# mederrata/spmf

Hardware: AMD Instinct MI355X
Metric: elbo_steps_per_sec (higher is better)
Workload: dtype f32

## Files before the change

### spmf_amd/csrc/common.h

```cpp
#pragma once
#include <hip/hip_runtime.h>
#include <stdint.h>

#define SPMF_WAVE 64

namespace spmf {

constexpr double kHalfLog2OverPi = -0.22579135264472743236;
constexpr double kLgammaHalf = 0.57236494292470008707;
constexpr double kLog2 = 0.69314718055994530942;

constexpr int kDaccHead = 6;
constexpr int kDaccDynSlot = 5;
__host__ __device__ constexpr bool lik_exp(int l) { return l == 1 || l == 4; }
__host__ __device__ constexpr bool lik_bern(int l) { return l == 2 || l == 4; }

constexpr float kYSat = 70.0f;
__device__ __forceinline__ float expm1_dec(float y, float& ey) {
  float p = 1.f / 40320.f;
  p = fmaf(p, y, 1.f / 5040.f);
  p = fmaf(p, y, 1.f / 720.f);
  p = fmaf(p, y, 1.f / 120.f);
  p = fmaf(p, y, 1.f / 24.f);
  p = fmaf(p, y, 1.f / 6.f);
  p = fmaf(p, y, 0.5f);
  p = fmaf(p, y, 1.f);
  const float e = expf(y);
  const bool small = fabsf(y) < 0.25f;
  const float em1 = small ? y * p : e - 1.f;
  ey = small ? 1.f + em1 : e;
  return em1;
}

__device__ __forceinline__ float cell_softplus(float r) { return fmaxf(r, 0.f) + log1pf(expf(-fabsf(r))); }
__device__ __forceinline__ bool cell_is_bern(int lik, const uint8_t* __restrict__ ctype, int d) {
  return lik_bern(lik) || (lik == 3 && ctype[d]);
}
__device__ __forceinline__ float cell_rate(int lik, float y, const float& phi, float& ey) {
  ey = 1.f;
  return (lik_exp(lik) ? expm1_dec(fminf(y, kYSat), ey) : y) + phi;
}
__device__ __forceinline__ float cell_ll0(bool bern, float r) { return bern ? -cell_softplus(r) : -r; }
template <bool LGAMMA>
__device__ __forceinline__ float cell_ll(bool bern, float x, float r) {
  if (bern) return x * r - cell_softplus(r);
  const float xl = x == 0.f ? 0.f : x * logf(r);
  return LGAMMA ? xl - lgammaf(x + 1.f) - r : xl - r;
}
__device__ __forceinline__ float cell_mean(bool bern, float r) {
  if (!bern) return r;
  const float e = expf(-fabsf(r));
  const float p = 1.f / (1.f + e);
  return r >= 0.f ? p : e * p;
}
__device__ __forceinline__ void lse_update(float ll, float& m, float& se) {
  const float d = ll - m;
  const float e = expf(-fabsf(d));
  se = d > 0.f ? fmaf(se, e, 1.f) : se + e;
  m = fmaxf(m, ll);
}

constexpr int kPrepSeg = 8;
#ifndef FINISH_FTD
#define FINISH_FTD 32
#endif
constexpr int kFinishCols = FINISH_FTD;
constexpr int kDaccRep = 16;
constexpr int kDetMaxBlocks = 4096;
constexpr int kDetMeta = 8;
__host__ __device__ inline int det_part_len(int KP) { return 2 * KP + 4; }

__host__ __device__ inline int acc_tail_len(int KP) { return 2 * (kDaccHead + KP); }
struct AccLayout {
  int D, KP, Dh;
  __host__ __device__ int64_t half_len(int h) const {
    return (int64_t)(h ? D - Dh : Dh) * (2 * KP + 1);
  }
  __host__ __device__ int64_t gA_off(int h) const { return h ? half_len(0) - (int64_t)Dh * KP : 0; }
  __host__ __device__ int64_t gV_off(int h) const {
    return h ? half_len(0) + (int64_t)(D - Dh) * KP - (int64_t)Dh * KP : (int64_t)Dh * KP;
  }
  __host__ __device__ int64_t gphi_off(int h) const {
    return h ? half_len(0) + (int64_t)2 * (D - Dh) * KP - Dh : (int64_t)2 * Dh * KP;
  }
  __host__ __device__ int64_t tail_off() const { return (int64_t)2 * D * KP + D; }
};
__host__ __device__ inline int64_t acc_len(int D, int KP) {
  return (int64_t)2 * D * KP + D + acc_tail_len(KP);
}

__device__ __forceinline__ void fold_dacc(int i, const double* __restrict__ dacc, float* __restrict__ tail, int KP) {
  double v = 0.0;
  if (i != kDaccDynSlot) {
#pragma unroll
    for (int r = 0; r < kDaccRep; ++r) v += dacc[(size_t)r * (kDaccHead + KP) + i];
  }
  const float hi = (float)v;
  tail[2 * i] = hi;
  tail[2 * i + 1] = (float)(v - (double)hi);
}

__device__ __forceinline__ double prep_sum(const double* __restrict__ dprep, int KP, int i) {
  double t = 0.0;
#pragma unroll
  for (int g = 0; g < kPrepSeg; ++g) t += dprep[(size_t)g * (KP + 1) + i];
  return t;
}

__device__ __forceinline__ float4 shfl4(float4 v, int src) {
  return make_float4(__shfl(v.x, src), __shfl(v.y, src), __shfl(v.z, src), __shfl(v.w, src));
}
__device__ __forceinline__ float4 shfl_xor4(float4 v, int m) {
  return make_float4(__shfl_xor(v.x, m), __shfl_xor(v.y, m), __shfl_xor(v.z, m),
                     __shfl_xor(v.w, m));
}
__device__ __forceinline__ float4 add4(float4 a, float4 b) {
  return make_float4(a.x + b.x, a.y + b.y, a.z + b.z, a.w + b.w);
}
__device__ __forceinline__ float4 fma4(float s, float4 a, float4 acc) {
  return make_float4(fmaf(s, a.x, acc.x), fmaf(s, a.y, acc.y), fmaf(s, a.z, acc.z),
                     fmaf(s, a.w, acc.w));
}
__device__ __forceinline__ float dot4(float4 a, float4 b) {
  return fmaf(a.x, b.x, fmaf(a.y, b.y, fmaf(a.z, b.z, a.w * b.w)));
}

template <int LPN>
__device__ __forceinline__ float4 gather4(const float* __restrict__ base, int row, int sub) {
  const uint32_t off = ((uint32_t)row * (uint32_t)LPN + (uint32_t)sub) * 16u;
  return *reinterpret_cast<const float4*>(reinterpret_cast<const char*>(base) + off);
}

constexpr int kPadRow = -1;
constexpr uint32_t kPadWord = 0xffff0000u;
struct GTable {
  __amdgpu_buffer_rsrc_t r;
};
__device__ __forceinline__ GTable gtable(const float* base, int64_t rows, int KP) {
  GTable t;
  t.r = __builtin_amdgcn_make_buffer_rsrc(const_cast<float*>(base), 0, (int)(uint32_t)((uint64_t)rows * KP * 4u),
                                          0x00020000);
  return t;
}
template <int LPN>
__device__ __forceinline__ float4 gather4(const GTable& t, int row, int sub) {
  const uint32_t off = ((uint32_t)row * (uint32_t)LPN + (uint32_t)sub) * 16u;
  typedef unsigned int u4 __attribute__((ext_vector_type(4)));
  const u4 v = __builtin_amdgcn_raw_buffer_load_b128(t.r, (int)off, 0, 0);
  return make_float4(__uint_as_float(v.x), __uint_as_float(v.y), __uint_as_float(v.z), __uint_as_float(v.w));
}

template <int CTRL>
__device__ __forceinline__ float dpp_add(float v) {
  const int t = __builtin_amdgcn_update_dpp(0, __float_as_int(v), CTRL, 0xF, 0xF, true);
  return v + __int_as_float(t);
}
template <int N>
__device__ __forceinline__ float group_sum(float v) {
  if constexpr (N >= 2) v = dpp_add<0xB1>(v);
  if constexpr (N >= 4) v = dpp_add<0x4E>(v);
  if constexpr (N >= 8) v = dpp_add<0x141>(v);
  if constexpr (N >= 16) v = dpp_add<0x140>(v);
  return v;
}
template <int LPN>
__device__ __forceinline__ float across_groups_sum(float v) {
  if constexpr (LPN <= 1) v = dpp_add<0x121>(v);
  if constexpr (LPN <= 2) v = dpp_add<0x122>(v);
  if constexpr (LPN <= 4) v = dpp_add<0x124>(v);
  if constexpr (LPN <= 8) v = dpp_add<0x128>(v);
  v += __shfl_xor(v, 16);
  v += __shfl_xor(v, 32);
  return v;
}
template <int LPN>
__device__ __forceinline__ float4 across_groups_sum4(float4 v) {
  return make_float4(across_groups_sum<LPN>(v.x), across_groups_sum<LPN>(v.y),
                     across_groups_sum<LPN>(v.z), across_groups_sum<LPN>(v.w));
}

__device__ __forceinline__ double wave_sum(double v) {
#pragma unroll
  for (int m = 32; m >= 1; m >>= 1) v += __shfl_xor(v, m);
  return v;
}
__device__ __forceinline__ float wave_sum(float v) {
#pragma unroll
  for (int m = 32; m >= 1; m >>= 1) v += __shfl_xor(v, m);
  return v;
}

__device__ __forceinline__ double block_sum(double v, double* red) {
  v = wave_sum(v);
  const int wid = threadIdx.x >> 6, lane = threadIdx.x & 63;
  const int nw = (blockDim.x + 63) >> 6;
  __syncthreads();
  if (lane == 0) red[wid] = v;
  __syncthreads();
  double t = 0.0;
  if (threadIdx.x == 0)
    for (int i = 0; i < nw; ++i) t += red[i];
  return t;
}

}
```

### spmf_amd/csrc/row_pass.hip

```cpp
#include <algorithm>

#include "common.h"
#include "kernels.h"

namespace spmf {

#ifndef ROW_MAX_BLOCKS
#define ROW_MAX_BLOCKS 4096
#endif
#ifndef ROW_DYN_NUM
#define ROW_DYN_NUM 1
#define ROW_DYN_DEN 8
#endif
static_assert(ROW_MAX_BLOCKS <= spmf::kDetMaxBlocks,
              "the deterministic mode's per-workgroup slots (common.h kDetMaxBlocks) are sized for at most that many row-pass workgroups");
#ifndef ROW_GRP
#define ROW_GRP 4
#endif
#ifndef ROW_V_AHEAD
#define ROW_V_AHEAD 2
#endif
#ifndef ROW_WAVES_PER_SIMD
#define ROW_WAVES_PER_SIMD 1
#endif

namespace {

__device__ __forceinline__ float* lds_dyn() {
  extern __shared__ __attribute__((aligned(16))) float spmf_row_lds[];
  return spmf_row_lds;
}

template <int FMT, bool NT>
__device__ __forceinline__ void load_entry(const int32_t* __restrict__ col, const float* __restrict__ val,
                                           const uint32_t* __restrict__ ent, int i, bool ok, int& ra,
                                           float& rb) {
  if (FMT == 1) {
    ra = ok ? (int)(NT ? __builtin_nontemporal_load(&ent[i]) : ent[i]) : (int)kPadWord;
    rb = 0.f;
  } else {
    ra = ok ? (NT ? __builtin_nontemporal_load(&col[i]) : col[i]) : kPadRow;
    rb = ok ? (NT ? __builtin_nontemporal_load(&val[i]) : val[i]) : 0.f;
  }
}
template <int FMT>
__device__ __forceinline__ void unpack_entry(int ra, float rb, int& c, float& x) {
  if (FMT == 1) {
    c = (int)((uint32_t)ra >> 16);
    x = (float)((uint32_t)ra & 0xffffu);
  } else {
    c = ra;
    x = rb;
  }
}

template <bool BASE>
__device__ __forceinline__ int bperm_i(int base_bytes, int imm_lanes, int v) {
  if constexpr (BASE) return __builtin_amdgcn_ds_bpermute(base_bytes + imm_lanes * 4, v);
  else return __shfl(v, (base_bytes >> 2) + imm_lanes);
}
template <bool BASE>
__device__ __forceinline__ float bperm_f(int base_bytes, int imm_lanes, float v) {
  return __int_as_float(bperm_i<BASE>(base_bytes, imm_lanes, __float_as_int(v)));
}

template <int KP, int LIK, bool LDSPHI = false>
struct RowCtx {
  static constexpr int LPN = KP / 4;
  static constexpr int NPI = 64 / LPN;
  static constexpr int GRP = LPN < ROW_GRP ? LPN : ROW_GRP;
  static constexpr bool BPI = LPN <= 8 && LIK != 1;
  GTable Ap, Vp;
  const float* phi;
  const uint8_t* ctype;
  int lane, sub, grp;
  int bp_grp, bp_row;

  template <int CNT>
  __device__ __forceinline__ void s1_group(int c, float x, int g0, float4& zacc) const {
    float4 a[CNT];
    float xv[CNT];
#pragma unroll
    for (int j = 0; j < CNT; ++j) {
      const int d = bperm_i<BPI>(bp_grp, (g0 + j) * NPI, c);
      xv[j] = bperm_f<BPI>(bp_grp, (g0 + j) * NPI, x);
      a[j] = gather4<LPN>(Ap, d, sub);
    }
#pragma unroll
    for (int j = 0; j < CNT; ++j) zacc = fma4(xv[j], a[j], zacc);
  }
  __device__ __forceinline__ void sweep1(int c, float x, int nchunk, float4& zacc) const {
#pragma unroll
    for (int g0 = 0; g0 < LPN; g0 += GRP) {
      if (g0 * NPI < nchunk) s1_group<GRP>(c, x, g0, zacc);
    }
  }

  template <int CNT>
  __device__ __forceinline__ void s2_gather(int c, int g0, const float4& z, float4 (&vv)[LPN],
                                            float& rmine) const {
#pragma unroll
    for (int j = 0; j < CNT; ++j) {
      const int d = bperm_i<BPI>(bp_grp, (g0 + j) * NPI, c);
      vv[g0 + j] = gather4<LPN>(Vp, d, sub);
    }
#pragma unroll
    for (int j = 0; j < CNT; ++j) {
      const float dot = group_sum<LPN>(dot4(z, vv[g0 + j]));
      if (sub == g0 + j) rmine = dot;
    }
#pragma unroll
    for (int j = CNT; j < GRP; ++j) vv[g0 + j] = make_float4(0.f, 0.f, 0.f, 0.f);
  }
  template <int CNT>
  __device__ __forceinline__ void s2_back(float cc, int g0, const float4 (&vv)[LPN],
                                          float4& gz) const {
#pragma unroll
    for (int j = 0; j < CNT; ++j) {
      const float cb = bperm_f<BPI>(bp_row, g0 + j, cc);
      gz = fma4(cb, vv[g0 + j], gz);
    }
  }

  __device__ __forceinline__ void s2_load(int c, int nchunk, float4 (&vv)[LPN]) const {
#pragma unroll
    for (int g0 = 0; g0 < LPN; g0 += GRP) {
      if (g0 * NPI < nchunk) {
#pragma unroll
        for (int j = 0; j < GRP; ++j) {
          const int d = bperm_i<BPI>(bp_grp, (g0 + j) * NPI, c);
          vv[g0 + j] = gather4<LPN>(Vp, d, sub);
        }
      } else {
#pragma unroll
        for (int j = 0; j < GRP; ++j) vv[g0 + j] = make_float4(0.f, 0.f, 0.f, 0.f);
      }
    }
  }
  __device__ __forceinline__ void sweep2_loaded(int c, float x, int nchunk, const float4& z, float4& gz, float& ll,
                                                double& nnf, const float4 (&vv)[LPN]) const {
    float rmine = 0.f;
#pragma unroll
    for (int g0 = 0; g0 < LPN; g0 += GRP) {
      if (g0 * NPI < nchunk) {
#pragma unroll
        for (int j = 0; j < GRP; ++j) {
          const float dot = group_sum<LPN>(dot4(z, vv[g0 + j]));
          if (sub == g0 + j) rmine = dot;
        }
      }
    }
    s2_cells(c, x, nchunk, rmine, vv, gz, ll, nnf);
  }

  __device__ __forceinline__ void sweep2(int c, float x, int nchunk, const float4& z,
                                         float4& gz, float& ll, double& nnf) const {
    float4 vv[LPN];
    float rmine = 0.f;
#pragma unroll
    for (int g0 = 0; g0 < LPN; g0 += GRP) {
      if (g0 * NPI < nchunk) s2_gather<GRP>(c, g0, z, vv, rmine);
      else s2_gather<0>(c, g0, z, vv, rmine);
    }
    s2_cells(c, x, nchunk, rmine, vv, gz, ll, nnf);
  }
  __device__ __forceinline__ void s2_cells(int c, float x, int nchunk, float rmine, const float4 (&vv)[LPN],
                                           float4& gz, float& ll, double& nnf) const {
    const int slot = sub * NPI + grp;
    const float xs = __shfl(x, slot);
    const int cs = __shfl(c, slot);
    float cc = 0.f;
    if (slot < nchunk && xs > 0.f) {
      if (LIK == 2 || LIK == 4 || (LIK == 3 && ctype[cs])) {
        float ey = 1.f;
        const float fy = LIK == 4 ? expm1_dec(fminf(rmine, kYSat), ey) : rmine;
        const float lg = fy + (LDSPHI ? lds_dyn()[cs] : phi[cs]);
        if (lg > -INFINITY && lg < INFINITY) {
          ll = fmaf(xs, lg, ll);
          cc = LIK == 4 ? xs * ey : xs;
        } else {
          nnf += 1.0;
        }
      } else {
        float ey = 1.f;
        const float fy = LIK == 1 ? expm1_dec(fminf(rmine, kYSat), ey) : rmine;
        const float r = fy + (LDSPHI ? lds_dyn()[cs] : phi[cs]);
        if (r > 0.f && r < INFINITY) {
          ll = fmaf(xs, logf(r), ll);
          cc = xs * ey * __builtin_amdgcn_rcpf(r);
        } else {
          nnf += 1.0;
          cc = ey;
        }
      }
    }
#pragma unroll
    for (int g0 = 0; g0 < LPN; g0 += GRP) {
      if (g0 * NPI < nchunk) s2_back<GRP>(cc, g0, vv, gz);
    }
  }
};

}

template <int KP, int LIK, int BT = 256, int PACKED = 0>
__global__ __launch_bounds__(BT, BT == 256 ? ROW_WAVES_PER_SIMD : 4) void row_pass_kernel(
    int64_t B, const int32_t* __restrict__ row_ptr, const int32_t* __restrict__ col,
    const float* __restrict__ val, const float* __restrict__ row_scale,
    const float* __restrict__ Ap, const float* __restrict__ Vp, const float* __restrict__ phi,
    const double* __restrict__ dprep, float* __restrict__ z, float* __restrict__ gzs,
    double* __restrict__ dacc, int mode, const float* __restrict__ gzd,
    const uint8_t* __restrict__ ctype, int Dcols, int64_t dacc_stride,
    const uint32_t* __restrict__ ent, double* __restrict__ det_slots, int64_t det_stride, int dyn_tail) {
  if (gridDim.y > 1) {
    const size_t sd = blockIdx.y;
    Ap += sd * (size_t)Dcols * KP;
    Vp += sd * (size_t)Dcols * KP;
    phi += sd * (size_t)Dcols;
    dprep += sd * (size_t)kPrepSeg * (KP + 1);
    z += sd * (size_t)B * KP;
    gzs += sd * (size_t)B * KP;
    dacc += sd * (size_t)dacc_stride;
  }
  const bool encode_only = mode == 1;
  constexpr int LPN = KP / 4;
  constexpr bool LDSPHI = BT != 256;
  if (LDSPHI && !encode_only) {
    float* pl = lds_dyn();
    for (int i = threadIdx.x; i < Dcols; i += BT) pl[i] = phi[i];
    __syncthreads();
  }
  RowCtx<KP, LIK, LDSPHI> cx;
  cx.Ap = gtable(Ap, Dcols, KP);
  cx.Vp = gtable(Vp, Dcols, KP);
  cx.phi = phi;
  cx.ctype = ctype;
  cx.lane = threadIdx.x & 63;
  cx.sub = cx.lane % LPN;
  cx.grp = cx.lane / LPN;
  cx.bp_grp = cx.grp * 4;
  cx.bp_row = cx.grp * LPN * 4;
  const int lane = cx.lane, sub = cx.sub, grp = cx.grp;
  const int64_t wave = ((int64_t)blockIdx.x * blockDim.x + threadIdx.x) >> 6;
  const int64_t nwaves = ((int64_t)gridDim.x * blockDim.x) >> 6;

  float4 veta4 = make_float4(0.f, 0.f, 0.f, 0.f);
  if (!encode_only && (mode != 2 || LIK == 3 || !gzd))
    veta4 = make_float4((float)prep_sum(dprep, KP, sub * 4 + 0), (float)prep_sum(dprep, KP, sub * 4 + 1),
                        (float)prep_sum(dprep, KP, sub * 4 + 2), (float)prep_sum(dprep, KP, sub * 4 + 3));
  double ll_acc = 0.0, zsq_acc = 0.0, nnf_acc = 0.0;
  float4 zsum = make_float4(0.f, 0.f, 0.f, 0.f);

  int64_t B_static = B;
  int64_t dyn_lo = B, dyn_hi = B;
  unsigned int* dyn_ctr = nullptr;
  if (dyn_tail && !det_slots && !encode_only) {
    const int64_t per_wave = B / nwaves;
    if (per_wave >= 8) {
      int64_t fixed = per_wave - (per_wave * ROW_DYN_NUM) / ROW_DYN_DEN;
      if (fixed < 2) fixed = 2;
      B_static = fixed * nwaves;
      const int r = (int)(wave & (kDaccRep - 1));
      const int64_t each = (B - B_static + kDaccRep - 1) / kDaccRep;
      dyn_lo = B_static + r * each;
      dyn_hi = dyn_lo + each < B ? dyn_lo + each : B;
      if (dyn_lo > B) dyn_lo = B;
      dyn_ctr = reinterpret_cast<unsigned int*>(dacc + (size_t)r * (kDaccHead + KP) + kDaccDynSlot);
    }
  }
  auto fixed_next = [&](int64_t cur) -> int64_t {
    if (cur >= B) return B;
    if (cur + nwaves < B_static) return cur + nwaves;
    return dyn_ctr ? (int64_t)-1 : B;
  };
  auto take_dynamic = [&]() -> int64_t {
    unsigned int k = 0;
    if (lane == 0) k = atomicAdd(dyn_ctr, 1u);
    k = (unsigned int)__builtin_amdgcn_readfirstlane((int)k);
    const int64_t row = dyn_lo + (int64_t)k;
    return row < dyn_hi ? row : B;
  };

  int start = 0, end = 0, pc0 = 0, pc1 = 0, nstart = 0, nend = 0;
  float xi = 1.f, px0 = 0.f, px1 = 0.f, nxi = 1.f;
  int64_t b = wave < B_static ? wave : B;
  int64_t bn = fixed_next(b);
  if (bn < 0) bn = take_dynamic();
  int64_t bnn = fixed_next(bn);
  if (bnn < 0) bnn = take_dynamic();
  if (b < B) {
    start = row_ptr[b];
    end = row_ptr[b + 1];
    xi = row_scale ? row_scale[b] : 1.f;
    const int f0 = min(end - start, 64);
    const int i0 = start + lane, i1 = start + f0 + lane;
    load_entry<PACKED, true>(col, val, ent, i0, lane < f0, pc0, px0);
    load_entry<PACKED, true>(col, val, ent, i1, i1 < end, pc1, px1);
  }
  if (bn < B) {
    nstart = row_ptr[bn];
    nend = row_ptr[bn + 1];
    nxi = row_scale ? row_scale[bn] : 1.f;
  }
  while (b < B) {
    const int n = end - start;
    int qc0 = 0, qc1 = 0, nnstart = 0, nnend = 0;
    float qx0 = 0.f, qx1 = 0.f, nnxi = 1.f;
    if (bn < B) {
      const int f0 = min(nend - nstart, 64);
      const int j0 = nstart + lane, j1 = nstart + f0 + lane;
      load_entry<PACKED, true>(col, val, ent, j0, lane < f0, qc0, qx0);
      load_entry<PACKED, true>(col, val, ent, j1, j1 < nend, qc1, qx1);
    }
    if (bnn < B) {
      nnstart = row_ptr[bnn];
      nnend = row_ptr[bnn + 1];
      nnxi = row_scale ? row_scale[bnn] : 1.f;
    }
    int64_t bnnn = fixed_next(bnn);
    unsigned int dyn_k = 0;
    const bool dyn_ask = bnnn < 0;
    if (dyn_ask && lane == 0) dyn_k = atomicAdd(dyn_ctr, 1u);
    float4 zacc = make_float4(0.f, 0.f, 0.f, 0.f);
    float4 gz = make_float4(0.f, 0.f, 0.f, 0.f);
    float llrow = 0.f;
    if (n <= 128) {
      int c0, c1;
      float x0, x1;
      unpack_entry<PACKED>(pc0, px0, c0, x0);
      unpack_entry<PACKED>(pc1, px1, c1, x1);
      const int n0 = min(n, 64), n1 = n - 64;
      constexpr int VAHEAD = KP <= 32 ? ROW_V_AHEAD : 0;
      float4 vv0[VAHEAD ? LPN : 1];
      if constexpr (VAHEAD == 1) {
        if (!encode_only) cx.s2_load(c0, n0, vv0);
      }
      if (mode != 2) {
        cx.sweep1(c0, x0, n0, zacc);
        if (n1 > 0) cx.sweep1(c1, x1, n1, zacc);
        if constexpr (VAHEAD == 3) {
          if (!encode_only) cx.s2_load(c0, n0, vv0);
        }
        zacc = across_groups_sum4<LPN>(zacc);
        zacc.x *= xi; zacc.y *= xi; zacc.z *= xi; zacc.w *= xi;
        if (grp == 0) reinterpret_cast<float4*>(z)[(size_t)b * LPN + sub] = zacc;
      } else {
        zacc = gather4<LPN>(z, (int)b, sub);
      }
      if (!encode_only) {
      if constexpr (VAHEAD != 0) {
        if constexpr (VAHEAD == 2) cx.s2_load(c0, n0, vv0);
        if constexpr (VAHEAD == 3) {
          if (mode == 2) cx.s2_load(c0, n0, vv0);
        }
        cx.sweep2_loaded(c0, x0, n0, zacc, gz, llrow, nnf_acc, vv0);
        if (n1 > 0) {
          float4 vv1[LPN];
          cx.s2_load(c1, n1, vv1);
          cx.sweep2_loaded(c1, x1, n1, zacc, gz, llrow, nnf_acc, vv1);
        }
      } else {
        cx.sweep2(c0, x0, n0, zacc, gz, llrow, nnf_acc);
        if (n1 > 0) cx.sweep2(c1, x1, n1, zacc, gz, llrow, nnf_acc);
      }
      }
    } else {
      if (mode != 2) {
        int ra = pc0, ra1 = pc1;
        float rb = px0, rb1 = px1;
        for (int base = start; base < end; base += 64) {
          const int i2 = base + 128 + lane;
          int ra2;
          float rb2;
          load_entry<PACKED, false>(col, val, ent, i2, i2 < end, ra2, rb2);
          int c;
          float x;
          unpack_entry<PACKED>(ra, rb, c, x);
          cx.sweep1(c, x, min(64, end - base), zacc);
          ra = ra1; rb = rb1; ra1 = ra2; rb1 = rb2;
        }
        zacc = across_groups_sum4<LPN>(zacc);
        zacc.x *= xi; zacc.y *= xi; zacc.z *= xi; zacc.w *= xi;
        if (grp == 0) reinterpret_cast<float4*>(z)[(size_t)b * LPN + sub] = zacc;
      } else {
        zacc = gather4<LPN>(z, (int)b, sub);
      }
      if (!encode_only) {
        int ra = pc0, ra1 = pc1;
        float rb = px0, rb1 = px1;
        for (int base = start; base < end; base += 64) {
          const int i2 = base + 128 + lane;
          int ra2;
          float rb2;
          load_entry<PACKED, false>(col, val, ent, i2, i2 < end, ra2, rb2);
          int c;
          float x;
          unpack_entry<PACKED>(ra, rb, c, x);
          cx.sweep2(c, x, min(64, end - base), zacc, gz, llrow, nnf_acc);
          ra = ra1; rb = rb1; ra1 = ra2; rb1 = rb2;
        }
      }
    }
    const float xi_cur = xi;
    const int64_t b_cur = b;
    start = nstart; end = nend; xi = nxi;
    pc0 = qc0; px0 = qx0; pc1 = qc1; px1 = qx1;
    nstart = nnstart; nend = nnend; nxi = nnxi;
    if (dyn_ask) {
      const int64_t row = dyn_lo + (int64_t)(unsigned int)__builtin_amdgcn_readfirstlane((int)dyn_k);
      bnnn = row < dyn_hi ? row : B;
    }
    b = bn; bn = bnn; bnn = bnnn;
    if (encode_only) continue;
    gz = across_groups_sum4<LPN>(gz);
    if (grp == 0) {
      zsq_acc += (double)dot4(zacc, zacc);
      zsum = add4(zsum, zacc);
      float4 dn = (mode == 2 && gzd) ? gather4<LPN>(gzd, (int)b_cur, sub) : veta4;
      if (LIK == 3 && mode == 2 && gzd) dn = add4(dn, veta4);
      if (mode == 3 && LIK != 3) dn = make_float4(0.f, 0.f, 0.f, 0.f);
      float4 o;
      o.x = xi_cur * (gz.x - dn.x - zacc.x);
      o.y = xi_cur * (gz.y - dn.y - zacc.y);
      o.z = xi_cur * (gz.z - dn.z - zacc.z);
      o.w = xi_cur * (gz.w - dn.w - zacc.w);
      reinterpret_cast<float4*>(gzs)[(size_t)b_cur * LPN + sub] = o;
    }
    ll_acc += (double)llrow;
  }
  if (encode_only) return;

  __shared__ double red[16];
  __shared__ double zred_static[BT == 256 ? 4 : 1][KP];
  if (LDSPHI) __syncthreads();
  double (*zred)[KP] = LDSPHI ? reinterpret_cast<double (*)[KP]>(lds_dyn()) : zred_static;
  const int wid = threadIdx.x >> 6;
  if (grp == 0) {
    zred[wid][sub * 4 + 0] = (double)zsum.x;
    zred[wid][sub * 4 + 1] = (double)zsum.y;
    zred[wid][sub * 4 + 2] = (double)zsum.z;
    zred[wid][sub * 4 + 3] = (double)zsum.w;
  }
  const double ll_b = block_sum(ll_acc, red);
  const double zq_b = block_sum(zsq_acc, red);
  const double nf_b = block_sum(nnf_acc, red);
  if (det_slots) {
    double* sl = det_slots + (size_t)blockIdx.y * det_stride;
    if (blockIdx.x == 0 && threadIdx.x == 0) sl[0] = (double)gridDim.x;
    sl += kDetMeta + (size_t)blockIdx.x * (kDaccHead + KP);
    if (threadIdx.x == 0) {
      sl[0] = ll_b;
      sl[1] = zq_b;
      sl[2] = nf_b;
      sl[3] = sl[4] = sl[5] = 0.0;
    }
    __syncthreads();
    if (threadIdx.x < KP) {
      double t = 0.0;
      const int nw = blockDim.x >> 6;
      for (int i = 0; i < nw; ++i) t += zred[i][threadIdx.x];
      sl[kDaccHead + threadIdx.x] = t;
    }
    return;
  }
  dacc += (size_t)(blockIdx.x % kDaccRep) * (kDaccHead + KP);
  if (threadIdx.x == 0) {
    atomicAdd(&dacc[0], ll_b);
    atomicAdd(&dacc[1], zq_b);
    if (nf_b != 0.0) atomicAdd(&dacc[2], nf_b);
  }
  __syncthreads();
  if (threadIdx.x < KP) {
    double t = 0.0;
    const int nw = blockDim.x >> 6;
    for (int i = 0; i < nw; ++i) t += zred[i][threadIdx.x];
    atomicAdd(&dacc[kDaccHead + threadIdx.x], t);
  }
}

template <int KP, int LIK, int BT, int PACKED>
static bool launch_row_lds_t(const RowArgs& a, hipStream_t st) {
  const size_t lds = a.mode == 1 ? 0 : std::max((size_t)a.D * 4, (size_t)(BT / 64) * KP * sizeof(double));
  constexpr int kMaxDev = 64;
  static size_t granted[kMaxDev] = {};
  if (lds > 64 * 1024) {
    int dev = 0;
    if (hipGetDevice(&dev) != hipSuccess || dev < 0 || dev >= kMaxDev) {
      (void)hipGetLastError();
      return false;
    }
    if (lds > __atomic_load_n(&granted[dev], __ATOMIC_RELAXED)) {
      if (hipFuncSetAttribute((const void*)row_pass_kernel<KP, LIK, BT, PACKED>,
                              hipFuncAttributeMaxDynamicSharedMemorySize, (int)lds) != hipSuccess) {
        (void)hipGetLastError();
        return false;
      }
      __atomic_store_n(&granted[dev], lds, __ATOMIC_RELAXED);
    }
  }
  const int64_t want = (a.B + (BT / 64) - 1) / (BT / 64);
#ifndef ROW_LDS_CAP
#define ROW_LDS_CAP 1024
#endif
  const int64_t cap = (int64_t)ROW_LDS_CAP * 256 / BT;
  const int nb = (int)(want < 1 ? 1 : (want > cap ? cap : want));
  hipLaunchKernelGGL((row_pass_kernel<KP, LIK, BT, PACKED>), dim3(nb, a.S > 1 ? a.S : 1), dim3(BT), lds, st,
                     a.B, a.row_ptr, a.col, a.val, a.row_scale, a.Ap, a.Vp, a.phi, a.dprep, a.z,
                     a.gzs, a.dacc, a.mode, a.gzd, a.ctype, a.D, a.dacc_stride, a.ent, a.det_slots, a.det_stride, a.dyn_tail);
  return true;
}

template <int KP, int LIK, int BT>
static bool launch_row_lds(const RowArgs& a, hipStream_t st) {
  return a.ent ? launch_row_lds_t<KP, LIK, BT, 1>(a, st) : launch_row_lds_t<KP, LIK, BT, 0>(a, st);
}

template <int KP>
static bool launch_row_t(const RowArgs& a, hipStream_t st) {
  int64_t want = (a.B + 3) / 4;
  int nb = (int)(want < 1 ? 1 : (want > ROW_MAX_BLOCKS ? ROW_MAX_BLOCKS : want));
  if constexpr (KP >= 16) {
    if (a.mode == 1 && a.B >= 4096) {
      if (launch_row_lds<KP, 0, 512>(a, st)) return true;
    }
    if (a.mode != 1 && a.logt >= 0 && a.logt <= 3 && a.B >= 4096) {
      const size_t need = (size_t)a.D * 4;
      bool done = false;
      if (need <= 80 * 1024) {
        done = a.logt == 0   ? launch_row_lds<KP, 0, 512>(a, st)
               : a.logt == 1 ? launch_row_lds<KP, 1, 512>(a, st)
               : a.logt == 2 ? launch_row_lds<KP, 2, 512>(a, st)
                             : launch_row_lds<KP, 3, 512>(a, st);
      } else if (need <= 160 * 1024 - 1024) {
        done = a.logt == 0   ? launch_row_lds<KP, 0, 1024>(a, st)
               : a.logt == 1 ? launch_row_lds<KP, 1, 1024>(a, st)
               : a.logt == 2 ? launch_row_lds<KP, 2, 1024>(a, st)
                             : launch_row_lds<KP, 3, 1024>(a, st);
      }
      if (done) return true;
    }
  }
#define SPMF_ROW_LAUNCH(L_)                                                                    \
  hipLaunchKernelGGL((row_pass_kernel<KP, L_>), dim3(nb, a.S > 1 ? a.S : 1), dim3(256), 0, st, \
                     a.B, a.row_ptr, a.col, a.val, a.row_scale, a.Ap, a.Vp, a.phi, a.dprep, a.z, \
                     a.gzs, a.dacc, a.mode, a.gzd, a.ctype, a.D, a.dacc_stride, a.ent, a.det_slots, a.det_stride, a.dyn_tail)
  if (a.logt == 4) SPMF_ROW_LAUNCH(4);
  else if (a.logt == 3) SPMF_ROW_LAUNCH(3);
  else if (a.logt == 2) SPMF_ROW_LAUNCH(2);
  else if (a.logt == 1) SPMF_ROW_LAUNCH(1);
  else SPMF_ROW_LAUNCH(0);
#undef SPMF_ROW_LAUNCH
  return true;
}

bool launch_row_pass(int KP, const RowArgs& a, hipStream_t st) {
  if (KP > 64) return launch_row_widek(KP, a, st);
  bool ok = false;
  return with_kp<64>(KP, [&](auto kp) { ok = launch_row_t<decltype(kp)::value>(a, st); }) && ok;
}

}
```

Measured before the change: 379.8.

## Issue next-row entry prefetch behind V gathers using buffer loads

Moves next-row entry loads, row_ptr fetches and the dynamic-tail atomic into a deferred issue_next hook. For KP<=32 it fires after the last V gather batch is issued, so those loads overlap the dot and cell math instead of stalling in front of it. Entry loads now use bounds-checked buffer resources rather than per-lane predicated loads, row_ptr/row_scale are read through the constant address space, and row indices are narrowed from int64 to int. It adds compiler-fence asm and an always-executed buffer atomic (zero-range resource when unused). It drops the ROW_V_AHEAD variants, so the register lifetimes and ordering of memory operations change.

```diff
diff --git a/spmf_amd/csrc/common.h b/spmf_amd/csrc/common.h
--- a/spmf_amd/csrc/common.h
+++ b/spmf_amd/csrc/common.h
@@ -150,6 +150,10 @@
   return make_float4(__uint_as_float(v.x), __uint_as_float(v.y), __uint_as_float(v.z), __uint_as_float(v.w));
 }
 
+__device__ __forceinline__ void issue_fence(const void* a, const void* b = nullptr, const void* c = nullptr) {
+  asm volatile("" ::"s"(a), "s"(b), "s"(c) : "memory");
+}
+
 template <int CTRL>
 __device__ __forceinline__ float dpp_add(float v) {
   const int t = __builtin_amdgcn_update_dpp(0, __float_as_int(v), CTRL, 0xF, 0xF, true);
diff --git a/spmf_amd/csrc/row_pass.hip b/spmf_amd/csrc/row_pass.hip
--- a/spmf_amd/csrc/row_pass.hip
+++ b/spmf_amd/csrc/row_pass.hip
@@ -17,9 +17,6 @@
 #ifndef ROW_GRP
 #define ROW_GRP 4
 #endif
-#ifndef ROW_V_AHEAD
-#define ROW_V_AHEAD 2
-#endif
 #ifndef ROW_WAVES_PER_SIMD
 #define ROW_WAVES_PER_SIMD 1
 #endif
@@ -31,26 +28,40 @@
   return spmf_row_lds;
 }
 
+template <int FMT>
+struct EntryRow {
+  __amdgpu_buffer_rsrc_t a, b;
+};
+template <int FMT>
+__device__ __forceinline__ EntryRow<FMT> entry_row(const int32_t* __restrict__ col, const float* __restrict__ val,
+                                                   const uint32_t* __restrict__ ent, int start, int n) {
+  EntryRow<FMT> r;
+  start = __builtin_amdgcn_readfirstlane(start);
+  n = __builtin_amdgcn_readfirstlane(n);
+  if (FMT == 1) {
+    r.a = __builtin_amdgcn_make_buffer_rsrc(const_cast<uint32_t*>(ent + start), 0, n * 4, 0x00020000);
+    r.b = r.a;
+  } else {
+    r.a = __builtin_amdgcn_make_buffer_rsrc(const_cast<int32_t*>(col + start), 0, n * 4, 0x00020000);
+    r.b = __builtin_amdgcn_make_buffer_rsrc(const_cast<float*>(val + start), 0, n * 4, 0x00020000);
+  }
+  return r;
+}
 template <int FMT, bool NT>
-__device__ __forceinline__ void load_entry(const int32_t* __restrict__ col, const float* __restrict__ val,
-                                           const uint32_t* __restrict__ ent, int i, bool ok, int& ra,
-                                           float& rb) {
+__device__ __forceinline__ void load_entry(const EntryRow<FMT>& r, int i, int& ra, float& rb) {
+  constexpr int AUX = NT ? 2 : 0;
+  ra = (int)__builtin_amdgcn_raw_buffer_load_b32(r.a, i * 4, 0, AUX);
+  rb = FMT == 1 ? 0.f : __uint_as_float(__builtin_amdgcn_raw_buffer_load_b32(r.b, i * 4, 0, AUX));
+}
+template <int FMT>
+__device__ __forceinline__ void unpack_entry(int ra, float rb, bool ok, int& c, float& x) {
   if (FMT == 1) {
-    ra = ok ? (int)(NT ? __builtin_nontemporal_load(&ent[i]) : ent[i]) : (int)kPadWord;
-    rb = 0.f;
+    const uint32_t w = ok ? (uint32_t)ra : kPadWord;
+    c = (int)(w >> 16);
+    x = (float)(w & 0xffffu);
   } else {
-    ra = ok ? (NT ? __builtin_nontemporal_load(&col[i]) : col[i]) : kPadRow;
-    rb = ok ? (NT ? __builtin_nontemporal_load(&val[i]) : val[i]) : 0.f;
-  }
-}
-template <int FMT>
-__device__ __forceinline__ void unpack_entry(int ra, float rb, int& c, float& x) {
-  if (FMT == 1) {
-    c = (int)((uint32_t)ra >> 16);
-    x = (float)((uint32_t)ra & 0xffffu);
-  } else {
-    c = ra;
-    x = rb;
+    c = ok ? ra : kPadRow;
+    x = ok ? rb : 0.f;
   }
 }
 
@@ -97,13 +108,15 @@
   }
 
   template <int CNT>
-  __device__ __forceinline__ void s2_gather(int c, int g0, const float4& z, float4 (&vv)[LPN],
-                                            float& rmine) const {
+  __device__ __forceinline__ void s2_issue(int c, int g0, float4 (&vv)[LPN]) const {
 #pragma unroll
     for (int j = 0; j < CNT; ++j) {
       const int d = bperm_i<BPI>(bp_grp, (g0 + j) * NPI, c);
       vv[g0 + j] = gather4<LPN>(Vp, d, sub);
     }
+  }
+  template <int CNT>
+  __device__ __forceinline__ void s2_dots(int g0, const float4& z, float4 (&vv)[LPN], float& rmine) const {
 #pragma unroll
     for (int j = 0; j < CNT; ++j) {
       const float dot = group_sum<LPN>(dot4(z, vv[g0 + j]));
@@ -153,14 +166,18 @@
     s2_cells(c, x, nchunk, rmine, vv, gz, ll, nnf);
   }
 
-  __device__ __forceinline__ void sweep2(int c, float x, int nchunk, const float4& z,
-                                         float4& gz, float& ll, double& nnf) const {
+  template <class Hook>
+  __device__ __forceinline__ void sweep2(int c, float x, int nchunk, const float4& z, float4& gz, float& ll,
+                                         double& nnf, Hook&& behind_last) const {
     float4 vv[LPN];
     float rmine = 0.f;
 #pragma unroll
     for (int g0 = 0; g0 < LPN; g0 += GRP) {
-      if (g0 * NPI < nchunk) s2_gather<GRP>(c, g0, z, vv, rmine);
-      else s2_gather<0>(c, g0, z, vv, rmine);
+      const bool occ = g0 * NPI < nchunk;
+      if (occ) s2_issue<GRP>(c, g0, vv);
+      if (g0 + GRP >= LPN) behind_last();
+      if (occ) s2_dots<GRP>(g0, z, vv, rmine);
+      else s2_dots<0>(g0, z, vv, rmine);
     }
     s2_cells(c, x, nchunk, rmine, vv, gz, ll, nnf);
   }
@@ -241,8 +258,9 @@
   cx.bp_grp = cx.grp * 4;
   cx.bp_row = cx.grp * LPN * 4;
   const int lane = cx.lane, sub = cx.sub, grp = cx.grp;
-  const int64_t wave = ((int64_t)blockIdx.x * blockDim.x + threadIdx.x) >> 6;
-  const int64_t nwaves = ((int64_t)gridDim.x * blockDim.x) >> 6;
+  const int wave = (int)blockIdx.x * (BT / 64) + __builtin_amdgcn_readfirstlane((int)(threadIdx.x >> 6));
+  const int nwaves = (int)gridDim.x * (BT / 64);
+  const int Bn = (int)B;
 
   float4 veta4 = make_float4(0.f, 0.f, 0.f, 0.f);
   if (!encode_only && (mode != 2 || LIK == 3 || !gzd))
@@ -251,120 +269,125 @@
   double ll_acc = 0.0, zsq_acc = 0.0, nnf_acc = 0.0;
   float4 zsum = make_float4(0.f, 0.f, 0.f, 0.f);
 
-  int64_t B_static = B;
-  int64_t dyn_lo = B, dyn_hi = B;
+  int B_static = Bn;
+  int dyn_lo = Bn, dyn_hi = Bn;
   unsigned int* dyn_ctr = nullptr;
   if (dyn_tail && !det_slots && !encode_only) {
-    const int64_t per_wave = B / nwaves;
+    const int per_wave = Bn / nwaves;
     if (per_wave >= 8) {
-      int64_t fixed = per_wave - (per_wave * ROW_DYN_NUM) / ROW_DYN_DEN;
+      int fixed = per_wave - (per_wave * ROW_DYN_NUM) / ROW_DYN_DEN;
       if (fixed < 2) fixed = 2;
       B_static = fixed * nwaves;
       const int r = (int)(wave & (kDaccRep - 1));
-      const int64_t each = (B - B_static + kDaccRep - 1) / kDaccRep;
+      const int each = (Bn - B_static + kDaccRep - 1) / kDaccRep;
       dyn_lo = B_static + r * each;
-      dyn_hi = dyn_lo + each < B ? dyn_lo + each : B;
-      if (dyn_lo > B) dyn_lo = B;
+      dyn_hi = dyn_lo + each < Bn ? dyn_lo + each : Bn;
+      if (dyn_lo > Bn) dyn_lo = Bn;
       dyn_ctr = reinterpret_cast<unsigned int*>(dacc + (size_t)r * (kDaccHead + KP) + kDaccDynSlot);
     }
   }
-  auto fixed_next = [&](int64_t cur) -> int64_t {
-    if (cur >= B) return B;
+  auto fixed_next = [&](int cur) -> int {
+    if (cur >= Bn) return Bn;
     if (cur + nwaves < B_static) return cur + nwaves;
-    return dyn_ctr ? (int64_t)-1 : B;
+    return dyn_ctr ? -1 : Bn;
   };
-  auto take_dynamic = [&]() -> int64_t {
+  auto take_dynamic = [&]() -> int {
     unsigned int k = 0;
     if (lane == 0) k = atomicAdd(dyn_ctr, 1u);
     k = (unsigned int)__builtin_amdgcn_readfirstlane((int)k);
-    const int64_t row = dyn_lo + (int64_t)k;
-    return row < dyn_hi ? row : B;
+    const int row = dyn_lo + (int)k;
+    return row < dyn_hi ? row : Bn;
   };
 
+  const __amdgpu_buffer_rsrc_t dyn_rsrc = __builtin_amdgcn_make_buffer_rsrc(
+      dyn_ctr ? dyn_ctr : reinterpret_cast<unsigned int*>(dacc), 0, dyn_ctr ? 4 : 0, 0x00020000);
+
+  typedef const __attribute__((address_space(4))) int32_t* RowPtr;
+  typedef const __attribute__((address_space(4))) float* RowScale;
+  const RowPtr rptr = (RowPtr)row_ptr;
+  const RowScale rscale = (RowScale)row_scale;
   int start = 0, end = 0, pc0 = 0, pc1 = 0, nstart = 0, nend = 0;
   float xi = 1.f, px0 = 0.f, px1 = 0.f, nxi = 1.f;
-  int64_t b = wave < B_static ? wave : B;
-  int64_t bn = fixed_next(b);
+  int b = wave < B_static ? wave : Bn;
+  int bn = fixed_next(b);
   if (bn < 0) bn = take_dynamic();
-  int64_t bnn = fixed_next(bn);
+  int bnn = fixed_next(bn);
   if (bnn < 0) bnn = take_dynamic();
-  if (b < B) {
-    start = row_ptr[b];
-    end = row_ptr[b + 1];
-    xi = row_scale ? row_scale[b] : 1.f;
-    const int f0 = min(end - start, 64);
-    const int i0 = start + lane, i1 = start + f0 + lane;
-    load_entry<PACKED, true>(col, val, ent, i0, lane < f0, pc0, px0);
-    load_entry<PACKED, true>(col, val, ent, i1, i1 < end, pc1, px1);
-  }
-  if (bn < B) {
-    nstart = row_ptr[bn];
-    nend = row_ptr[bn + 1];
-    nxi = row_scale ? row_scale[bn] : 1.f;
-  }
-  while (b < B) {
+  if (b < Bn) {
+    start = rptr[b];
+    end = rptr[b + 1];
+    xi = row_scale ? rscale[b] : 1.f;
+    const EntryRow<PACKED> er = entry_row<PACKED>(col, val, ent, start, end - start);
+    load_entry<PACKED, true>(er, lane, pc0, px0);
+    load_entry<PACKED, true>(er, lane + 64, pc1, px1);
+  }
+  if (bn < Bn) {
+    nstart = rptr[bn];
+    nend = rptr[bn + 1];
+    nxi = row_scale ? rscale[bn] : 1.f;
+  }
+  while (b < Bn) {
     const int n = end - start;
     int qc0 = 0, qc1 = 0, nnstart = 0, nnend = 0;
     float qx0 = 0.f, qx1 = 0.f, nnxi = 1.f;
-    if (bn < B) {
-      const int f0 = min(nend - nstart, 64);
-      const int j0 = nstart + lane, j1 = nstart + f0 + lane;
-      load_entry<PACKED, true>(col, val, ent, j0, lane < f0, qc0, qx0);
-      load_entry<PACKED, true>(col, val, ent, j1, j1 < nend, qc1, qx1);
-    }
-    if (bnn < B) {
-      nnstart = row_ptr[bnn];
-      nnend = row_ptr[bnn + 1];
-      nnxi = row_scale ? row_scale[bnn] : 1.f;
-    }
-    int64_t bnnn = fixed_next(bnn);
+    int bnnn = fixed_next(bnn);
+    const bool dyn_ask = bnnn < 0;
     unsigned int dyn_k = 0;
-    const bool dyn_ask = bnnn < 0;
-    if (dyn_ask && lane == 0) dyn_k = atomicAdd(dyn_ctr, 1u);
+    auto issue_next = [&]() {
+      issue_fence(PACKED ? (const void*)ent : (const void*)col, val, row_ptr);
+      dyn_k = (unsigned int)__builtin_amdgcn_raw_ptr_buffer_atomic_add_i32(1, dyn_rsrc, (dyn_ask && lane == 0) ? 0 : 4,
+                                                                       0, 0);
+      const EntryRow<PACKED> er = entry_row<PACKED>(col, val, ent, nstart, nend - nstart);
+      load_entry<PACKED, true>(er, lane, qc0, qx0);
+      load_entry<PACKED, true>(er, lane + 64, qc1, qx1);
+      if (bnn < Bn) {
+        nnstart = rptr[bnn];
+        nnend = rptr[bnn + 1];
+        nnxi = row_scale ? rscale[bnn] : 1.f;
+      }
+      issue_fence(PACKED ? (const void*)ent : (const void*)col, val, row_ptr);
+    };
+    constexpr bool BEHIND = KP <= 32;
+    if constexpr (!BEHIND) issue_next();
     float4 zacc = make_float4(0.f, 0.f, 0.f, 0.f);
     float4 gz = make_float4(0.f, 0.f, 0.f, 0.f);
     float llrow = 0.f;
     if (n <= 128) {
       int c0, c1;
       float x0, x1;
-      unpack_entry<PACKED>(pc0, px0, c0, x0);
-      unpack_entry<PACKED>(pc1, px1, c1, x1);
-      const int n0 = min(n, 64), n1 = n - 64;
-      constexpr int VAHEAD = KP <= 32 ? ROW_V_AHEAD : 0;
-      float4 vv0[VAHEAD ? LPN : 1];
-      if constexpr (VAHEAD == 1) {
-        if (!encode_only) cx.s2_load(c0, n0, vv0);
-      }
+      unpack_entry<PACKED>(pc0, px0, lane < n, c0, x0);
+      unpack_entry<PACKED>(pc1, px1, lane + 64 < n, c1, x1);
+      int n0 = min(n, 64);
+      const int n1 = n - 64;
       if (mode != 2) {
         cx.sweep1(c0, x0, n0, zacc);
         if (n1 > 0) cx.sweep1(c1, x1, n1, zacc);
-        if constexpr (VAHEAD == 3) {
-          if (!encode_only) cx.s2_load(c0, n0, vv0);
-        }
         zacc = across_groups_sum4<LPN>(zacc);
         zacc.x *= xi; zacc.y *= xi; zacc.z *= xi; zacc.w *= xi;
         if (grp == 0) reinterpret_cast<float4*>(z)[(size_t)b * LPN + sub] = zacc;
       } else {
         zacc = gather4<LPN>(z, (int)b, sub);
       }
-      if (!encode_only) {
-      if constexpr (VAHEAD != 0) {
-        if constexpr (VAHEAD == 2) cx.s2_load(c0, n0, vv0);
-        if constexpr (VAHEAD == 3) {
-          if (mode == 2) cx.s2_load(c0, n0, vv0);
-        }
-        cx.sweep2_loaded(c0, x0, n0, zacc, gz, llrow, nnf_acc, vv0);
-        if (n1 > 0) {
-          float4 vv1[LPN];
-          cx.s2_load(c1, n1, vv1);
-          cx.sweep2_loaded(c1, x1, n1, zacc, gz, llrow, nnf_acc, vv1);
-        }
+      if (encode_only) {
+        if constexpr (BEHIND) issue_next();
       } else {
-        cx.sweep2(c0, x0, n0, zacc, gz, llrow, nnf_acc);
-        if (n1 > 0) cx.sweep2(c1, x1, n1, zacc, gz, llrow, nnf_acc);
-      }
+        if constexpr (KP <= 32) {
+          float4 vv[LPN];
+          if (n1 > 0) {
+            cx.s2_load(c0, n0, vv);
+            cx.sweep2_loaded(c0, x0, n0, zacc, gz, llrow, nnf_acc, vv);
+            c0 = c1; x0 = x1; n0 = n1;
+          }
+          cx.s2_load(c0, n0, vv);
+          issue_next();
+          cx.sweep2_loaded(c0, x0, n0, zacc, gz, llrow, nnf_acc, vv);
+        } else {
+          cx.sweep2(c0, x0, n0, zacc, gz, llrow, nnf_acc, [] {});
+          if (n1 > 0) cx.sweep2(c1, x1, n1, zacc, gz, llrow, nnf_acc, [] {});
+        }
       }
     } else {
+      const EntryRow<PACKED> er = entry_row<PACKED>(col, val, ent, start, n);
       if (mode != 2) {
         int ra = pc0, ra1 = pc1;
         float rb = px0, rb1 = px1;
@@ -372,10 +395,10 @@
           const int i2 = base + 128 + lane;
           int ra2;
           float rb2;
-          load_entry<PACKED, false>(col, val, ent, i2, i2 < end, ra2, rb2);
+          load_entry<PACKED, false>(er, i2 - start, ra2, rb2);
           int c;
           float x;
-          unpack_entry<PACKED>(ra, rb, c, x);
+          unpack_entry<PACKED>(ra, rb, base + lane < end, c, x);
           cx.sweep1(c, x, min(64, end - base), zacc);
           ra = ra1; rb = rb1; ra1 = ra2; rb1 = rb2;
         }
@@ -385,30 +408,33 @@
       } else {
         zacc = gather4<LPN>(z, (int)b, sub);
       }
-      if (!encode_only) {
+      if (encode_only) {
+        if constexpr (BEHIND) issue_next();
+      } else {
         int ra = pc0, ra1 = pc1;
         float rb = px0, rb1 = px1;
         for (int base = start; base < end; base += 64) {
           const int i2 = base + 128 + lane;
           int ra2;
           float rb2;
-          load_entry<PACKED, false>(col, val, ent, i2, i2 < end, ra2, rb2);
+          load_entry<PACKED, false>(er, i2 - start, ra2, rb2);
           int c;
           float x;
-          unpack_entry<PACKED>(ra, rb, c, x);
-          cx.sweep2(c, x, min(64, end - base), zacc, gz, llrow, nnf_acc);
+          unpack_entry<PACKED>(ra, rb, base + lane < end, c, x);
+          if (BEHIND && base + 64 >= end) cx.sweep2(c, x, end - base, zacc, gz, llrow, nnf_acc, issue_next);
+          else cx.sweep2(c, x, min(64, end - base), zacc, gz, llrow, nnf_acc, [] {});
           ra = ra1; rb = rb1; ra1 = ra2; rb1 = rb2;
         }
       }
     }
     const float xi_cur = xi;
-    const int64_t b_cur = b;
+    const int b_cur = b;
     start = nstart; end = nend; xi = nxi;
     pc0 = qc0; px0 = qx0; pc1 = qc1; px1 = qx1;
     nstart = nnstart; nend = nnend; nxi = nnxi;
-    if (dyn_ask) {
-      const int64_t row = dyn_lo + (int64_t)(unsigned int)__builtin_amdgcn_readfirstlane((int)dyn_k);
-      bnnn = row < dyn_hi ? row : B;
+    {
+      const int row = dyn_lo + (int)(unsigned int)__builtin_amdgcn_readfirstlane((int)dyn_k);
+      if (dyn_ask) bnnn = row < dyn_hi ? row : Bn;
     }
     b = bn; bn = bnn; bnn = bnnn;
     if (encode_only) continue;
```

Result: faster. 386.5, median of 6 (+1.8%).
